# PhiSpel/lettuce

Measured on AMD Instinct MI355X. Metric: MLUPS (million lattice updates/s) D3Q19 256³ TGV; achieved HBM GB/s vs peak, higher is better.
Workload: dtype f32; 1 GPU; TaylorGreenVortex3D D3Q19 BGK fp32 256x256x256 (16777216 nodes per GPU), Re=1600 Ma=0.1; parallelism=single GPU

## Files before the change

### lettuce_amd/csrc/api.hip

```cpp
#include <hip/hip_runtime.h>
#include <stdarg.h>
#include <stdio.h>
#include <string.h>

#include <algorithm>
#include <cmath>
#include <new>
#include <type_traits>

#include "dispatch.hpp"
#include "kernels.hpp"
#include "lettuce_hip.h"

namespace {

thread_local char g_error[512] = "";

int fail(int code, const char *fmt, ...) {
  va_list ap;
  va_start(ap, fmt);
  vsnprintf(g_error, sizeof g_error, fmt, ap);
  va_end(ap);
  return code;
}
// ... 1250 lines not shown
  return aux(p, 0, f, nullptr, u0, nullptr, s, 1.0, 1.0, nullptr, (owned + 6) * plane);
}
int lt_slab_enstrophy(lt_plan *p, const void *u_ext, double u_scale, double inv_dx, double *out, void *s) {
  if (const int rc = slab_plan_ok(p, "lt_slab_enstrophy")) return rc;
  if (!out || !u_ext) return fail(LT_ERR_INVALID, "null output / velocity field");
  return aux(p, 8, nullptr, nullptr, const_cast<void *>(u_ext), out, s, u_scale, inv_dx);
}
int lt_slab_mass_interior(lt_plan *p, const void *f, const uint8_t *mask, int32_t z_begin, int32_t nz_global,
                          double *out, void *s) {
  if (const int rc = slab_plan_ok(p, "lt_slab_mass_interior")) return rc;
  if (!out) return fail(LT_ERR_INVALID, "null output");
  const int owned = p->interior_end - p->interior_begin;
  if (z_begin < 0 || nz_global < 1 || z_begin + owned > nz_global)
    return fail(LT_ERR_INVALID, "planes [%d, %d) of %d", z_begin, z_begin + owned, nz_global);
  return aux(p, 9, f, nullptr, nullptr, out, s, 1.0, 1.0, mask, 0, z_begin, nz_global);
}

int lt_plan_kernel_info(lt_plan *p, int32_t *vec, int32_t *tpb, int64_t *blocks) {
  if (!p) return fail(LT_ERR_INVALID, "null plan");
  if (vec) *vec = 1;
  if (tpb) *tpb = lt::kThreads;
  if (blocks) {
    const long long nodes = (long long)p->n0 * p->n1 * (p->interior_end - p->interior_begin);
    *blocks = (nodes + lt::kThreads - 1) / lt::kThreads;
  }
  return LT_OK;
}

const char *lt_plan_kernel_name(lt_plan *p) {
  if (!p) return "";
  int mode = (two_step_wanted(p) || p->desc.ghost_planes == 2) ? lt::kFusedTwice : lt::kFused;
  if (many_step_wanted(p)) mode = lt::kFusedMany;
  if (mode == lt::kFusedTwice && !has_kernel(p->unit, kernel_selector(p, mode))) mode = lt::kFused;
  const lt::StepArgs a = kernel_selector(p, mode);
  if (!p->unit.name(a, lt::NameBuf{p->kernel_name, sizeof p->kernel_name})) p->kernel_name[0] = 0;
  return p->kernel_name;
}

int lt_slab_crossing(lt_plan *p, int32_t direction, int32_t *q_out, int32_t *n_out) {
  if (!p || !n_out) return fail(LT_ERR_INVALID, "null argument");
  const lt::QList ql = crossing(p, direction);
  *n_out = ql.n;
  if (q_out) for (int k = 0; k < ql.n; ++k) q_out[k] = ql.q[k];
  return LT_OK;
}
int lt_slab_pack(lt_plan *p, const void *f, int64_t plane, int32_t direction, void *buf, void *s) {
  return pack(p, true, const_cast<void *>(f), plane, direction, buf, s);
}
int lt_slab_unpack(lt_plan *p, void *f, int64_t plane, int32_t direction, const void *buf, void *s) {
  return pack(p, false, f, plane, direction, const_cast<void *>(buf), s);
}

int lt_probe_copy(void *dst, const void *src, int64_t n_bytes, int32_t cache_policy,
                  int32_t max_blocks, void *stream) {
  if (!dst || !src || n_bytes < 16 || n_bytes % 16 != 0 || (uintptr_t)dst % 16 || (uintptr_t)src % 16)
    return fail(LT_ERR_INVALID, "probe copy needs 16-byte aligned buffers and size");
  const size_t n = (size_t)n_bytes / 16;
  size_t grid = (n + 255) / 256;
  if (max_blocks > 0 && grid > (size_t)max_blocks) grid = (size_t)max_blocks;
  hipStream_t s = static_cast<hipStream_t>(stream);
  const probe_f4 *sp = static_cast<const probe_f4 *>(src);
  probe_f4 *dp = static_cast<probe_f4 *>(dst);
  switch (cache_policy) {
    case 0: hipLaunchKernelGGL(probe_copy_kernel<0>, dim3((unsigned)grid), dim3(256), 0, s, sp, dp, n); break;
    case 1: hipLaunchKernelGGL(probe_copy_kernel<1>, dim3((unsigned)grid), dim3(256), 0, s, sp, dp, n); break;
    case 2: hipLaunchKernelGGL(probe_copy_kernel<2>, dim3((unsigned)grid), dim3(256), 0, s, sp, dp, n); break;
    case 3: hipLaunchKernelGGL(probe_copy_kernel<3>, dim3((unsigned)grid), dim3(256), 0, s, sp, dp, n); break;
// ... 494 lines not shown
```

### lettuce_amd/csrc/dispatch.hpp

```cpp
#pragma once
#include <hip/hip_runtime.h>
#include <stddef.h>
#include <stdint.h>

namespace lt {

enum StepMode { kFused = 0, kCollideOnly = 1, kStreamOnly = 2, kFusedTwice = 3, kFusedMany = 4 };

constexpr int kCollNone = 0, kCollBgk = 1, kCollKbc = 2, kCollSmagorinsky = 3, kCollForce = 4, kCollTrt = 8,
              kCollRegularized = 9, kCollMrt = 10, kCollMrtLallemand = 11;
constexpr int kCollIncompressible = 16;
constexpr bool coll_incompressible(int coll) { return (coll & kCollIncompressible) != 0; }
constexpr bool coll_mrt(int coll) { return coll == kCollMrt || coll == kCollMrtLallemand; }
constexpr bool coll_forced(int coll) {
  return (coll & ~kCollIncompressible) == (kCollBgk | kCollForce) || coll == (kCollSmagorinsky | kCollForce);
}
constexpr int coll_base(int coll) { return coll_forced(coll) ? coll & ~kCollForce : coll; }

struct StepArgs {
  const void *in;
  void *out;
  int n0, n1, n2;
  long long stride_in, stride_out;
  int p_begin, planes;
// ... 65 lines not shown
#define LT_UNIT_d3q19_f32 D3Q19, float,  19, 3, 0, 1
#define LT_UNIT_d3q19_f64 D3Q19, double, 19, 3, 0, 0
#define LT_UNIT_d3q27_f32 D3Q27, float,  27, 3, 1, 0
#define LT_UNIT_d3q27_f64 D3Q27, double, 27, 3, 1, 0
#define LT_UNIT_d1q3_f32  D1Q3,  float,   3, 1, 0, 0
#define LT_UNIT_d1q3_f64  D1Q3,  double,  3, 1, 0, 0
#define LT_UNIT_d3q15_f32 D3Q15, float,  15, 3, 0, 0
#define LT_UNIT_d3q15_f64 D3Q15, double, 15, 3, 0, 0
#define LT_UNITS(X)                                                                                  \
  X(d2q9_f32) X(d2q9_f64) X(d3q19_f32) X(d3q19_f64) X(d3q27_f32) X(d3q27_f64) X(d1q3_f32) X(d1q3_f64) \
  X(d3q15_f32) X(d3q15_f64)
#define LT_FIELD(name, tag) LT_FIELD_A(name, tag)
#define LT_FIELD_A(name, tag) LT_FIELD_B(name, LT_UNIT_##tag)
#define LT_FIELD_B(name, ...) LT_FIELD_##name(__VA_ARGS__)
#define LT_FIELD_lattice(s, t, q, d, kbc, roles) s
#define LT_FIELD_scalar(s, t, q, d, kbc, roles) t
#define LT_FIELD_q(s, t, q, d, kbc, roles) q
#define LT_FIELD_d(s, t, q, d, kbc, roles) d
#define LT_FIELD_kbc(s, t, q, d, kbc, roles) kbc
#define LT_FIELD_roles(s, t, q, d, kbc, roles) roles

#define LT_DECLARE_UNIT(tag)                                   \
  int step_##tag(const StepArgs &);                            \
  int aux_##tag(const AuxArgs &);                              \
  const char *name_##tag(const StepArgs &, const NameBuf &);   \
  int forced_##tag(const StepArgs &, const NameBuf *);         \
  int relax_##tag(const StepArgs &, const NameBuf *);          \
  int outlets_##tag(const StepArgs &, const NameBuf *);        \
  int outlets2_##tag(const StepArgs &, const NameBuf *);       \
  int outlets3_##tag(const StepArgs &, const NameBuf *);       \
  int twice_##tag(const StepArgs &, const NameBuf *);          \
  int smag_##tag(const StepArgs &, const NameBuf *);           \
  int roles_##tag(const StepArgs &, const NameBuf *);          \
  int mrt_##tag(const StepArgs &, const NameBuf *);            \
  int mrt_outlets_##tag(const StepArgs &, const NameBuf *);    \
  int incompressible_##tag(const StepArgs &, const NameBuf *); \
  int incompressible_aux_##tag(const AuxArgs &);               \
  int spectrum_##tag(const AuxArgs &);
LT_UNITS(LT_DECLARE_UNIT)

constexpr int kNoKernel = -1;

}
```

### lettuce_amd/csrc/kernels.hpp

```cpp
#pragma once
#include <hip/hip_runtime.h>
#include <stdint.h>

#include "dispatch.hpp"
#include "lattice.hpp"
#include "mrt.hpp"
#include "twostep_roles.hpp"

namespace lt {

constexpr int kThreads = 256;
constexpr int kMaxB = 127;

constexpr int kBounceBack = 1, kEquilibrium = 2, kAbbOutlet = 3;
constexpr int kPressureOutlet = 4;
constexpr int kOutletsP = 4;

template <typename T>
struct BoundaryTable {
  int kind[kMaxB + 1];
  int mem_axis[kMaxB + 1];
  int side[kMaxB + 1];
  int plane[kMaxB + 1];
  int nbr[kMaxB + 1];
// ... 959 lines not shown
  static_assert(VEC == 1 && SHIFT == 0, "one node per thread");
  static_assert(coll_incompressible(COLL) && !coll_forced(COLL), "the incompressible equilibrium is COLL & 16");
  lbm_body<T, S, LAYOUT, COLL, STREAM, COLLIDE, MASKED, TUNE, PACK, ABBD>(p);
}
template <typename T, class S, int LAYOUT, int COLL, bool STREAM, bool COLLIDE, bool MASKED,
          int VEC, int SHIFT, int TUNE = 0, bool PACK = false, int ABBD = 0>
__global__ void __launch_bounds__(kThreads) lbm_kernel(const KParamsFI<T> p) {
  static_assert(VEC == 1 && SHIFT == 0, "one node per thread");
  static_assert(coll_incompressible(COLL) && coll_forced(COLL), "BGK with a body force and the incompressible equilibrium is COLL 21");
  lbm_body<T, S, LAYOUT, COLL, STREAM, COLLIDE, MASKED, TUNE, PACK, ABBD>(p);
}

template <typename T, class S, int LAYOUT, int COLL, bool STREAM, bool COLLIDE, bool MASKED,
          int VEC, int SHIFT, int TUNE = 0, bool PACK = false>
__global__ void __launch_bounds__(kThreads, 4) lbm_kernel_occ4(const KParams<T> p) {
  static_assert(VEC == 1 && SHIFT == 0, "one node per thread");
  lbm_body<T, S, LAYOUT, COLL, STREAM, COLLIDE, MASKED, TUNE, PACK>(p);
}

template <typename T, class S, int T0_, int T1>
struct TwoStep {
  static constexpr int T0 = T0_, H0 = T0 + 2, H1 = T1 + 2;
  static constexpr int NI = H0 * H1;
  static constexpr int NO = T0 * T1;
  static constexpr int THREADS = (NI + 63) / 64 * 64;
  template <int LAYOUT, int E2>
  static constexpr int count() {
    int n = 0;
    for (int q = 0; q < S::Q; ++q) n += MemMap<S, LAYOUT>::e(q, 2) == E2 ? 1 : 0;
    return n;
  }
};

__device__ __forceinline__ void lds_barrier() {
  asm volatile("s_waitcnt lgkmcnt(0)\n\ts_barrier" ::: "memory");
}

template <typename T, class S, int LAYOUT, int COLL, int T0_, int T1, int NPT = 1, int MODE = 0,
          int NPB = NPT, int SCHED = 0>
__global__ void __launch_bounds__((SCHED == 0 ? (TwoStep<T, S, T0_, T1>::NI / NPT + 63) / 64 * 64
                                              : RoleWaves<TwoStep<T, S, T0_, T1>::NI, TwoStep<T, S, T0_, T1>::NO>::THREADS))
lbm2_kernel(const KParams<T> p, const int seg_len) {
  static_assert(!coll_forced(COLL), "kernels with a body force take KParamsF");
#include "twostep_sweep.inc"
}

template <typename T, class S, int LAYOUT, int COLL, int T0_, int T1, int NPT = 1, int MODE = 0,
          int NPB = NPT, int SCHED = 0>
__global__ void __launch_bounds__((TwoStep<T, S, T0_, T1>::NI / NPT + 63) / 64 * 64)
lbm2_kernel(const KParamsF<T> p, const int seg_len) {
  static_assert(coll_forced(COLL), "a body force exists for BGK (5) and Smagorinsky (7)");
#include "twostep_sweep.inc"
}

static __global__ void wait_counter_kernel(const unsigned long long *counter, unsigned long long target,
                                           unsigned *timed_out) {
  const long long t0 = wall_clock64();
  while (__hip_atomic_load(counter, __ATOMIC_RELAXED, __HIP_MEMORY_SCOPE_AGENT) < target) {
    __builtin_amdgcn_s_sleep(127);
    if (wall_clock64() - t0 > 100000000ll) {
      *timed_out = 1u;
      break;
    }
  }
  __atomic_thread_fence(__ATOMIC_ACQUIRE);
}
// ... 447 lines not shown
```

### lettuce_amd/csrc/twostep_masked.hpp

```cpp
#pragma once
#include "kernels.hpp"

namespace lt {

typedef unsigned bufu2 __attribute__((ext_vector_type(2)));

template <typename T> struct BufIO;
template <> struct BufIO<float> {
  static __device__ __forceinline__ float load(__amdgpu_buffer_rsrc_t r, unsigned voff, unsigned soff) {
    return __builtin_bit_cast(float, __builtin_amdgcn_raw_buffer_load_b32(r, (int)voff, (int)soff, 0));
  }
  static __device__ __forceinline__ void store_nt(float v, __amdgpu_buffer_rsrc_t r, unsigned voff, unsigned soff) {
    __builtin_amdgcn_raw_buffer_store_b32(__builtin_bit_cast(unsigned, v), r, (int)voff, (int)soff, 2);
  }
};
template <> struct BufIO<double> {
  static __device__ __forceinline__ double load(__amdgpu_buffer_rsrc_t r, unsigned voff, unsigned soff) {
    return __builtin_bit_cast(double, __builtin_amdgcn_raw_buffer_load_b64(r, (int)voff, (int)soff, 0));
  }
  static __device__ __forceinline__ void store_nt(double v, __amdgpu_buffer_rsrc_t r, unsigned voff, unsigned soff) {
    __builtin_amdgcn_raw_buffer_store_b64(__builtin_bit_cast(bufu2, v), r, (int)voff, (int)soff, 2);
  }
};

template <typename T>
__device__ __forceinline__ __amdgpu_buffer_rsrc_t field_rsrc(const T *field, unsigned bytes) {
  return __builtin_amdgcn_make_buffer_rsrc(const_cast<T *>(field), 0, (int)bytes, 0x00020000);
}

constexpr int kEqCached = 2;
template <typename T, class S, int LAYOUT, int T0, int T1>
constexpr size_t two_step_masked_lds() {
  using B = TwoStep<T, S, T0, T1>;
  return sizeof(T) * ((size_t)B::NI * (4 * B::template count<LAYOUT, 1>() + 3 * B::template count<LAYOUT, 0>() +
                                       3 * B::template count<LAYOUT, -1>()) + (size_t)kEqCached * S::Q);
}

struct MaskedPlanInfo {
  unsigned kinds;
  unsigned fields;
  int eq0, eq1;
  int abb_slot, abb_side, abb_plane, abb_axis;
};
template <typename T>
__device__ __forceinline__ MaskedPlanInfo masked_plan_info(const KParams<T> &p) {
  MaskedPlanInfo m = {0u, 0u, 0, 0, 0, 1, -1, 2};
  int cached = 0;
  for (int slot = 1; slot <= p.nb; ++slot) {
    const int kind = p.bt->kind[slot];
    m.kinds |= (unsigned)kind << (2 * slot);
    if (kind == kEquilibrium) {
      if (p.bt->field[slot]) m.fields |= 1u << slot;
      else if (cached == 0) { m.eq0 = slot; cached = 1; }
      else if (cached == 1) { m.eq1 = slot; cached = 2; }
    }
    if (kind == kAbbOutlet) {
      m.abb_slot = slot; m.abb_side = p.bt->side[slot]; m.abb_plane = p.bt->plane[slot];
      m.abb_axis = p.bt->mem_axis[slot];
    }
  }
  return m;
// ... 302 lines not shown
```

### lettuce_amd/csrc/twostep_roles.hpp

```cpp
#pragma once
#include <type_traits>

#if defined(__HIPCC__)
#define LT_ROLE_FN __host__ __device__ __forceinline__
#else
#define LT_ROLE_FN inline
#endif

namespace lt {

template <int SET>
using RegSet = std::integral_constant<int, SET>;

template <class Load, class Fill, class Sync, class Drain, class Emit>
LT_ROLE_FN void role_sweep(const int s, const int last, Load &&load, Fill &&fill, Sync &&sync, Drain &&drain,
                           Emit &&emit) {
  load(s - 1, RegSet<0>{});
  load(s, RegSet<1>{});
  fill(0, 0, RegSet<0>{});
  load(s + 1, RegSet<0>{});
  fill(1, 1, RegSet<1>{});
  int k = s, r = 1, r3 = 1;
  auto interval = [&](auto cur, auto with_load, auto with_fill) {
    constexpr int CUR = decltype(cur)::value;
// ... 4 lines not shown
    emit(k);
    ++k;
    ++r;
    r3 = r3 == 2 ? 0 : r3 + 1;
  };
  using Yes = std::true_type;
  using No = std::false_type;
  if (s + 2 > last) {
    fill(2, 2, RegSet<0>{});
    interval(RegSet<1>{}, No{}, No{});
    return;
  }
  load(s + 2, RegSet<1>{});
  fill(2, 2, RegSet<0>{});
  for (;;) {
    if (k + 3 > last) { interval(RegSet<1>{}, No{}, Yes{}); break; }
    interval(RegSet<1>{}, Yes{}, Yes{});
    if (k + 3 > last) { interval(RegSet<0>{}, No{}, Yes{}); break; }
    interval(RegSet<0>{}, Yes{}, Yes{});
  }
  while (k < last) interval(RegSet<0>{}, No{}, No{});
}

template <int NI, int NO>
struct RoleWaves {
  static constexpr int PW = (NI + 63) / 64;
  static constexpr int CPB = PW + NO / 64 > 16 ? 2 : 1;
  static constexpr int CW = NO / CPB / 64;
  static constexpr int THREADS = (PW + CW) * 64;
  static_assert(NO % (CPB * 64) == 0, "whole consumer waves");
  static_assert(PW + CW <= 16, "a workgroup has at most 1024 threads");
};

}
```

### lettuce_amd/csrc/twostep_sweep.inc

```
  constexpr bool PACK = MODE == 1;
  static_assert(MODE == 0 || LAYOUT == 1, "edge / signalling launches exist in the slab layout");
  static_assert(NPT == 1 && NPB == 1, "one intermediate and one output node per thread");
  static_assert(SCHED == 0 || (SCHED == 1 && MODE == 0), "separate producer and consumer waves: the plain sweep");
  using B = TwoStep<T, S, T0_, T1>;
  using M = MemMap<S, LAYOUT>;
  constexpr int T0 = B::T0, H0 = B::H0, NI = B::NI, NO = B::NO;
  constexpr int NU = B::template count<LAYOUT, 1>(), NC = B::template count<LAYOUT, 0>(),
                ND = B::template count<LAYOUT, -1>();
  static_assert(COLL == kCollNone || COLL == kCollBgk || COLL == kCollSmagorinsky || coll_forced(COLL) || COLL == kCollTrt ||
                    COLL == kCollRegularized,
                "two-step kernel: streaming only, BGK or Smagorinsky, the latter two also with a body force, TRT, regularised");
  static_assert(COLL == kCollNone || COLL == kCollBgk || (SCHED == 0 && MODE == 0),
                "Smagorinsky, body force, TRT, regularised: the plain one-role sweep only");
  __shared__ T lds_u[4][NU][NI];
  __shared__ T lds_c[3][NC][NI];
  __shared__ T lds_d[2][ND][NI];

  const int tid = threadIdx.x;
  const int tiles0 = p.n0 / T0, tiles1 = p.n1 / T1;
  int b = blockIdx.x;
  const int segs_a = (p.p_end - p.p_begin + seg_len - 1) / seg_len;
  if (MODE == 2) {
    const int tiles = tiles0 * tiles1;
    const int layer = b / tiles, t = b - layer * tiles;
    const int tile = tiles % 8 == 0 ? (t % 8) * (tiles / 8) + t / 8 : t;
    b = (layer == 0 ? segs_a : layer - 1) * tiles + tile;
  } else if (p.nb == 0 && (tiles0 * tiles1) % 8 == 0) {
    const int tiles = tiles0 * tiles1;
    const int layer = b / tiles, t = b - layer * tiles;
    b = layer * tiles + (t % 8) * (tiles / 8) + t / 8;
  } else if (p.nb != 1 && gridDim.x % 8 == 0) {
    b = (b % 8) * (gridDim.x / 8) + b / 8;
  }
  const int t0 = (b % tiles0) * T0; b /= tiles0;
  const int t1 = (b % tiles1) * T1; b /= tiles1;
  const bool second = b >= segs_a;
// ... 4 lines not shown
  unsigned voff[NPT][3][3];
  unsigned out_off[NPB];
  int a_at[NPT];
  int b_at[NPB];
  static_for<NPT>([&](auto kc) {
    constexpr int k = decltype(kc)::value;
    const int ia = tid + k * NI;
    constexpr int inner = T0 * B::H1;
    const int i1 = ia < inner ? ia / T0 : (ia - inner) >> 1;
    const int i0 = ia < inner ? 1 + (ia - i1 * T0) : (((ia - inner) & 1) ? H0 - 1 : 0);
    a_at[k] = i1 * H0 + i0;
    int g0 = t0 + i0 - 1; g0 = g0 < 0 ? g0 + p.n0 : (g0 >= p.n0 ? g0 - p.n0 : g0);
    int g1 = t1 + i1 - 1; g1 = g1 < 0 ? g1 + p.n1 : (g1 >= p.n1 ? g1 - p.n1 : g1);
    const int g0m = g0 == 0 ? p.n0 - 1 : g0 - 1, g0p = g0 == p.n0 - 1 ? 0 : g0 + 1;
    const int g1m = g1 == 0 ? p.n1 - 1 : g1 - 1, g1p = g1 == p.n1 - 1 ? 0 : g1 + 1;
#pragma unroll
    for (int a = 0; a < 3; ++a)
#pragma unroll
      for (int c = 0; c < 3; ++c) {
        const int y = a == 0 ? g1p : (a == 1 ? g1 : g1m);
        const int x = c == 0 ? g0p : (c == 1 ? g0 : g0m);
        voff[k][a][c] = ((unsigned)y * (unsigned)p.n0 + (unsigned)x) * (unsigned)sizeof(T);
      }
  });
  static_for<NPB>([&](auto kc) {
    constexpr int k = decltype(kc)::value;
    const int ib = tid + k * NO;
    const int j1 = ib / T0, j0 = ib - j1 * T0;
    out_off[k] = ((unsigned)(t1 + j1) * (unsigned)p.n0 + (unsigned)(t0 + j0)) * (unsigned)sizeof(T);
    b_at[k] = (j1 + 1) * H0 + (j0 + 1);
  });
  const unsigned plane_nodes = (unsigned)p.n1 * (unsigned)p.n0;

  if constexpr (SCHED == 1) {
    using R = RoleWaves<NI, NO>;
    constexpr int CPB = R::CPB, CT = NO / CPB;
    const int last = s + seg_len < range_end ? s + seg_len : range_end;
    auto sync = [&]() { lds_barrier(); };
    if (__builtin_amdgcn_readfirstlane(tid >> 6) < R::PW) {
      if (!in_a) {
#pragma unroll
        for (int a = 0; a < 3; ++a)
#pragma unroll
          for (int c = 0; c < 3; ++c) voff[0][a][c] = 0u;
      }
      T set0[S::Q][1], set1[S::Q][1];
      auto load = [&](int plane, auto set) {
        T (&dst)[S::Q][1] = decltype(set)::value == 0 ? set0 : set1;
        int g2 = plane, g2m = plane - 1, g2p = plane + 1;
        if (p.wrap2) {
          g2 = plane < 0 ? plane + p.n2 : (plane >= p.n2 ? plane - p.n2 : plane);
          g2m = g2 == 0 ? p.n2 - 1 : g2 - 1;
          g2p = g2 == p.n2 - 1 ? 0 : g2 + 1;
        }
        static_for<S::Q>([&](auto qc) {
          constexpr int q = decltype(qc)::value;
          constexpr int e0 = M::e(q, 0), e1 = M::e(q, 1), e2 = M::e(q, 2);
          const int z = e2 == 0 ? g2 : (e2 > 0 ? g2m : g2p);
          const T *base = p.in + ((long long)q * p.Ni + (long long)((unsigned)z * plane_nodes));
          dst[q][0] = *reinterpret_cast<const T *>(reinterpret_cast<const char *>(base) + voff[0][e1 + 1][e0 + 1]);
        });
        __builtin_amdgcn_sched_barrier(0);
      };
      auto fill = [&](int r, int r3, auto set) {
        T (&src)[S::Q][1] = decltype(set)::value == 0 ? set0 : set1;
        collide_node<T, S, LAYOUT, 1, 0, COLL>(src, p);
        if (in_a) {
          static_for<S::Q>([&](auto qc) {
            constexpr int q = decltype(qc)::value;
            constexpr int e2 = M::e(q, 2), rank = crossing_rank<S, LAYOUT, q>();
            if constexpr (e2 > 0) lds_u[r & 3][rank][a_at[0]] = src[q][0];
            else if constexpr (e2 == 0) lds_c[r3][rank][a_at[0]] = src[q][0];
            else lds_d[r & 1][rank][a_at[0]] = src[q][0];
          });
        }
        __builtin_amdgcn_sched_barrier(0);
      };
      role_sweep(s, last, load, fill, sync, [](int, int) {}, [](int) {});
    } else {
      const int c = tid - R::PW * 64;
      unsigned c_off[CPB];
      int c_at[CPB];
      static_for<CPB>([&](auto kc) {
        constexpr int k = decltype(kc)::value;
        const int ib = c + k * CT;
        const int j1 = ib / T0, j0 = ib - j1 * T0;
        c_off[k] = ((unsigned)(t1 + j1) * (unsigned)p.n0 + (unsigned)(t0 + j0)) * (unsigned)sizeof(T);
        c_at[k] = (j1 + 1) * H0 + (j0 + 1);
      });
      T f[S::Q][CPB];
      auto drain = [&](int r, int r3) {
        static_for<S::Q>([&](auto qc) {
          constexpr int q = decltype(qc)::value;
          constexpr int e0 = M::e(q, 0), e1 = M::e(q, 1), e2 = M::e(q, 2), rank = crossing_rank<S, LAYOUT, q>();
          static_for<CPB>([&](auto kc) {
            constexpr int k = decltype(kc)::value;
            const int at = c_at[k] - e1 * H0 - e0;
            if constexpr (e2 > 0) f[q][k] = lds_u[(r - 1) & 3][rank][at];
            else if constexpr (e2 == 0) f[q][k] = lds_c[r3][rank][at];
            else f[q][k] = lds_d[(r + 1) & 1][rank][at];
          });
        });
      };
      auto emit = [&](int k2) {
        static_for<CPB>([&](auto kc) { collide_node<T, S, LAYOUT, CPB, decltype(kc)::value, COLL>(f, p); });
        static_for<S::Q>([&](auto qc) {
          constexpr int q = decltype(qc)::value;
          T *base = p.out + ((long long)q * p.No + (long long)((unsigned)k2 * plane_nodes));
          static_for<CPB>([&](auto kc) {
            constexpr int k = decltype(kc)::value;
            __builtin_nontemporal_store(f[q][k], reinterpret_cast<T *>(reinterpret_cast<char *>(base) + c_off[k]));
          });
        });
      };
      role_sweep(s, last, [](int, auto) {}, [](int, int, auto) {}, sync, drain, emit);
    }
    return;
  }
  T pre[S::Q][NPT];
  auto load_a = [&](int plane) {
    int g2 = plane, g2m = plane - 1, g2p = plane + 1;
    if (p.wrap2) {
      g2 = plane < 0 ? plane + p.n2 : (plane >= p.n2 ? plane - p.n2 : plane);
      g2m = g2 == 0 ? p.n2 - 1 : g2 - 1;
      g2p = g2 == p.n2 - 1 ? 0 : g2 + 1;
    }
    if (in_a) {
      static_for<S::Q>([&](auto qc) {
        constexpr int q = decltype(qc)::value;
        constexpr int e0 = M::e(q, 0), e1 = M::e(q, 1), e2 = M::e(q, 2);
        const int z = e2 == 0 ? g2 : (e2 > 0 ? g2m : g2p);
        const T *base = p.in + ((long long)q * p.Ni + (long long)((unsigned)z * plane_nodes));
        if constexpr (MODE == 1) {
          constexpr int rank = crossing_rank<S, LAYOUT, q>();
          if constexpr (e2 >= 0) {
            if (p.ghost_lo != nullptr && z < p.lo)
              base = p.ghost_lo + (size_t)(e2 == 0 ? rank : (z == p.lo - 1 ? NC + rank : NC + NU + rank)) * plane_nodes;
          }
          if constexpr (e2 <= 0) {
            if (p.ghost_hi != nullptr && z >= p.hi)
              base = p.ghost_hi + (size_t)(e2 == 0 ? rank : (z == p.hi ? NC + rank : NC + ND + rank)) * plane_nodes;
          }
        }
        static_for<NPT>([&](auto kc) {
          constexpr int k = decltype(kc)::value;
// ... 189 lines not shown
```

### lettuce_amd/csrc/unit.inc

```
#include <cstdio>
#include <algorithm>
#include <type_traits>

#include "dispatch.hpp"
#include "kernels.hpp"
#include "twostep_masked.hpp"
#include "twostep2d.hpp"
#include "spectrum.hpp"

#define LT_CAT_(a, b) a##b
#define LT_CAT(a, b) LT_CAT_(a, b)
#define LT_TAG LT_UNIT
#define LT_S lt::LT_FIELD(lattice, LT_UNIT)
#define LT_T LT_FIELD(scalar, LT_UNIT)
#define LT_IS_3D (LT_FIELD(d, LT_UNIT) == 3)
#define LT_HAS_KBC LT_FIELD(kbc, LT_UNIT)
#define LT_HAS_ROLES LT_FIELD(roles, LT_UNIT)
#define LT_HAS_MRT (LT_FIELD(q, LT_UNIT) == 9 || LT_FIELD(q, LT_UNIT) == 27)

#define LT_PART_main 1
#define LT_PART_sweeps 2
#define LT_PART_roles 3
#define LT_PART_smagorinsky 4
#define LT_PART_forced 5
#define LT_PART_relaxations 6
#define LT_PART_outlets 7
#define LT_PART_outlets2 8
#define LT_PART_outlets3 9
#define LT_PART_mrt 10
#define LT_PART_mrt_outlets 11
#define LT_PART_incompressible 12
#define LT_PART_spectrum 13
#define LT_PART_IS_OUTLETS (LT_PART_IS(outlets) || LT_PART_IS(outlets2) || LT_PART_IS(outlets3) || LT_PART_IS(mrt_outlets))
#define LT_PART_IS(name) (LT_CAT(LT_PART_, LT_PART) == LT_PART_##name)
#if LT_PART_IS(main)
#define LT_ONE_STEP 1
#define LT_SWEEP 0
#elif LT_PART_IS(sweeps)
#define LT_ONE_STEP 0
#define LT_SWEEP 1
#elif LT_PART_IS(roles)
#define LT_ONE_STEP 0
#define LT_SWEEP 1
#elif LT_PART_IS(smagorinsky)
#define LT_ONE_STEP 1
#define LT_SWEEP 0
#elif LT_PART_IS(forced)
#define LT_ONE_STEP 1
#define LT_SWEEP 1
#elif LT_PART_IS(relaxations)
#define LT_ONE_STEP 1
#define LT_SWEEP 1
#elif LT_PART_IS_OUTLETS || LT_PART_IS(mrt) || LT_PART_IS(incompressible)
#define LT_ONE_STEP 1
#define LT_SWEEP 0
#elif LT_PART_IS(spectrum)
#define LT_ONE_STEP 0
#define LT_SWEEP 0
#else
#error "LT_PART: main, sweeps, roles, smagorinsky, forced, relaxations, outlets, outlets2, outlets3, mrt, mrt_outlets, incompressible or spectrum"
#endif
#if (LT_PART_IS(mrt) || LT_PART_IS(mrt_outlets)) && !LT_HAS_MRT
#error "the MRT collision exists on D2Q9 and D3Q27"
#endif
#if LT_PART_IS(spectrum) && LT_FIELD(d, LT_UNIT) < 2
#error "the energy spectrum exists in 2-D and 3-D"
#endif

namespace lt {
namespace {

using S = LT_S;
using T = LT_T;
constexpr size_t kTwicePerNode = sizeof(T) * 3 * S::Q;
constexpr int kTwiceW = 256 / (int)sizeof(T);
constexpr int kTwiceR = kTwicePerNode * (kTwiceW + 2) * 10 <= 160 * 1024 ? 8
                        : (sizeof(T) == 4 && kTwicePerNode * (kTwiceW + 2) * 6 <= 160 * 1024 ? 4 : 0);

template <int COLL>
using ParamsOfQuadratic = std::conditional_t<coll_mrt(COLL), KParamsM<T>, std::conditional_t<coll_forced(COLL), KParamsF<T>, KParams<T>>>;
template <int COLL>
using ParamsOf = std::conditional_t<coll_incompressible(COLL), std::conditional_t<coll_forced(COLL), KParamsFI<T>, KParamsI<T>>,
                                    ParamsOfQuadratic<COLL>>;
template <class P>
P params_of(const StepArgs &a, int n2) {
  P p{};
  p.in = static_cast<const T *>(a.in);
  p.out = static_cast<T *>(a.out);
  p.n0 = a.n0; p.n1 = a.n1; p.n2 = n2;
  p.nv0 = a.n0;
  p.p_begin = a.p_begin;
  p.p_stride = a.p_stride;
  p.wrap2 = a.wrap2;
// ... 168 lines not shown
  return kNoKernel;
}
#endif

#endif

#if LT_SWEEP
template <int LAYOUT, int COLL, int T0, int T1, int MODE = 0, int SCHED = 0>
int launch_twice(const StepArgs &a, const NameBuf *name) {
  if constexpr (S::D == 3 && T0 > 0 &&
                (COLL == kCollNone || COLL == kCollBgk ||
                 ((COLL == kCollSmagorinsky || COLL == (kCollBgk | kCollForce) || COLL == kCollTrt || COLL == kCollRegularized) &&
                  S::Q == 19 && sizeof(T) == 4 && MODE == 0 && SCHED == 0))) {
    using B = TwoStep<T, S, T0, T1>;
    if (name) return kernel_name(*name, "lbm2_kernel", LAYOUT, COLL, T0, T1, 1, MODE, 1, elided(SCHED));
    if (a.n0 % T0 != 0 || a.n1 % T1 != 0 || a.seg_len < 1 || a.masked || a.planes < 1 || a.p_stride != 1 ||
        (long long)a.n0 * a.n1 * (long long)sizeof(T) >= (1ll << 32))
      return kNoKernel;
    if (MODE == 2 && (!a.signal || a.planes2 < 2 || a.planes2 > a.seg_len || a.seg_len < 2)) return kNoKernel;
    using P = ParamsOf<COLL>;
    P p = params_of<P>(a, a.n2);
    p.p_end = a.p_begin + a.planes;
    p.p_begin2 = a.p_begin2;
    p.p_end2 = a.p_begin2 + a.planes2;
    if constexpr (coll_forced(COLL)) set_force<LAYOUT>(p, a);
    p.nb = a.shift == 3 ? 1 : (a.shift == 4 ? 2 : 0);
    p.signal = MODE == 2 ? a.signal : nullptr;
    p.edge_first = MODE == 2 ? 1 : 0;
    p.ghost_lo = static_cast<const T *>(a.ghost_lo);
    p.ghost_hi = static_cast<const T *>(a.ghost_hi);
    p.lo = a.interior_begin; p.hi = a.interior_end;
    const unsigned grid = (unsigned)((a.n0 / T0) * (a.n1 / T1) * ((a.planes + a.seg_len - 1) / a.seg_len +
                                                                   (a.planes2 + a.seg_len - 1) / a.seg_len));
    constexpr int threads = SCHED ? RoleWaves<B::NI, B::NO>::THREADS : (B::NI + 63) / 64 * 64;
    void (*kern)(const P, const int) = lbm2_kernel<T, S, LAYOUT, COLL, T0, T1, 1, MODE, 1, SCHED>;
    hipLaunchKernelGGL(kern, dim3(grid), dim3(threads), 0, a.stream, p, a.seg_len);
    return (int)hipGetLastError();
  } else {
    return kNoKernel;
  }
}

int sweep(const StepArgs &a, const NameBuf *name) {
  constexpr int W = kTwiceW, R = kTwiceR;
  if constexpr (R > 0) {
#if LT_PART_IS(roles)
    if (a.layout == 0) return launch_twice<0, kCollBgk, W, R, 0, 1>(a, name);
    return launch_twice<1, kCollBgk, W, R, 0, 1>(a, name);
#elif LT_PART_IS(forced)
    if (a.masked || a.pack_lo || a.pack_hi || a.signal) return kNoKernel;
    if (a.layout == 0 && a.coll == (kCollBgk | kCollForce)) return launch_twice<0, kCollBgk | kCollForce, W, R>(a, name);
    if (a.layout == 1 && a.coll == (kCollBgk | kCollForce)) return launch_twice<1, kCollBgk | kCollForce, W, R>(a, name);
#elif LT_PART_IS(relaxations)
    if (a.masked || a.pack_lo || a.pack_hi || a.signal) return kNoKernel;
    if (a.layout == 0 && a.coll == kCollTrt) return launch_twice<0, kCollTrt, W, R>(a, name);
    if (a.layout == 1 && a.coll == kCollTrt) return launch_twice<1, kCollTrt, W, R>(a, name);
    if (a.layout == 0 && a.coll == kCollRegularized) return launch_twice<0, kCollRegularized, W, R>(a, name);
    if (a.layout == 1 && a.coll == kCollRegularized) return launch_twice<1, kCollRegularized, W, R>(a, name);
#else
    const int coll = a.coll;
#if LT_HAS_ROLES
    if (coll == kCollBgk && a.shift != 6 && (a.layout == 0 || !(a.pack_lo || a.pack_hi || a.signal)))
      return LT_CAT(roles_, LT_TAG)(a, name);
#endif
    if (a.layout == 0 && coll == kCollNone) return launch_twice<0, kCollNone, W, R>(a, name);
    if (a.layout == 0 && coll == kCollBgk) return launch_twice<0, kCollBgk, W, R>(a, name);
    if (a.layout == 0 && coll == kCollSmagorinsky) return launch_twice<0, kCollSmagorinsky, W, R>(a, name);
    if (coll == kCollSmagorinsky && (a.pack_lo || a.pack_hi || a.signal)) return kNoKernel;
    if (a.layout == 1 && (a.pack_lo || a.pack_hi)) {
      if (coll == kCollNone) return launch_twice<1, kCollNone, W, R, 1>(a, name);
      if (coll == kCollBgk) return launch_twice<1, kCollBgk, W, R, 1>(a, name);
    }
    if (a.layout == 1 && a.signal) {
      if (coll == kCollNone) return launch_twice<1, kCollNone, W, R, 2>(a, name);
      if (coll == kCollBgk) return launch_twice<1, kCollBgk, W, R, 2>(a, name);
    }
    if (a.layout == 1 && coll == kCollNone) return launch_twice<1, kCollNone, W, R>(a, name);
    if (a.layout == 1 && coll == kCollBgk) return launch_twice<1, kCollBgk, W, R>(a, name);
    if (a.layout == 1 && coll == kCollSmagorinsky) return launch_twice<1, kCollSmagorinsky, W, R>(a, name);
#endif
  }
// ... 242 lines not shown
        hipLaunchKernelGGL(finish_sum_kernel<false>, dim3(1), dim3(kThreads), 0, a.stream, a.partial,
                           a.reduce_blocks, a.out);
        break;
      } else {
        return kNoKernel;
      }
    default:
      return kNoKernel;
  }
  return (int)hipGetLastError();
}

#endif

}

#if LT_PART_IS(main)
int LT_CAT(step_, LT_TAG)(const StepArgs &a) { return dispatch(a, nullptr); }

const char *LT_CAT(name_, LT_TAG)(const StepArgs &a, const NameBuf &name) {
  return dispatch(a, &name) == 0 ? name.s : nullptr;
}

int LT_CAT(aux_, LT_TAG)(const AuxArgs &a) {
#if LT_IS_3D
  if (a.layout == 1) return aux_impl<1>(a);
#endif
  return aux_impl<0>(a);
}
#elif LT_PART_IS(sweeps)
int LT_CAT(twice_, LT_TAG)(const StepArgs &a, const NameBuf *name) { return sweep(a, name); }
#elif LT_PART_IS(roles)
int LT_CAT(roles_, LT_TAG)(const StepArgs &a, const NameBuf *name) { return sweep(a, name); }
#elif LT_PART_IS(smagorinsky)
int LT_CAT(smag_, LT_TAG)(const StepArgs &a, const NameBuf *name) { return one_step_of<kCollSmagorinsky>(a, name); }
#elif LT_PART_IS(forced)
int LT_CAT(forced_, LT_TAG)(const StepArgs &a, const NameBuf *name) {
  if (a.mode == kFusedTwice) return S::D == 3 ? sweep(a, name) : kNoKernel;
  if (a.coll == (kCollBgk | kCollForce)) return one_step_of<kCollBgk | kCollForce>(a, name);
  if (a.coll == (kCollSmagorinsky | kCollForce)) return one_step_of<kCollSmagorinsky | kCollForce>(a, name);
  return kNoKernel;
}
#elif LT_PART_IS(relaxations)
int LT_CAT(relax_, LT_TAG)(const StepArgs &a, const NameBuf *name) {
  if (a.mode == kFusedTwice) return S::D == 3 ? sweep(a, name) : kNoKernel;
  if (a.mode != kFused && a.mode != kCollideOnly) return kNoKernel;
  if (a.coll == kCollTrt) return one_step_of<kCollTrt>(a, name);
  if (a.coll == kCollRegularized) return one_step_of<kCollRegularized>(a, name);
  return kNoKernel;
}
#elif LT_PART_IS(outlets)
int LT_CAT(outlets_, LT_TAG)(const StepArgs &a, const NameBuf *name) {
  if (a.mode != kFused && a.mode != kCollideOnly) return kNoKernel;
  switch (a.coll) {
    case kCollNone: return pressure_outlets_of<kCollNone>(a, name);
    case kCollBgk: return pressure_outlets_of<kCollBgk>(a, name);
#if LT_HAS_KBC
    case kCollKbc: return pressure_outlets_of<kCollKbc>(a, name);
#endif
    case kCollSmagorinsky: case kCollTrt: case kCollRegularized: return LT_CAT(outlets2_, LT_TAG)(a, name);
    case kCollBgk | kCollForce: case kCollSmagorinsky | kCollForce: return LT_CAT(outlets3_, LT_TAG)(a, name);
#if LT_HAS_MRT
    case kCollMrt: case kCollMrtLallemand: return LT_CAT(mrt_outlets_, LT_TAG)(a, name);
#endif
    default: return kNoKernel;
  }
// ... 76 lines not shown
```

Baseline: 68680 MLUPS.

## Use buffer loads/stores and trimmed LDS writes in role-split two-step BGK sweep

For the producer/consumer role-split two-step kernel in the SoA layout, global loads and non-temporal stores now go through AMD buffer resources with scalar (uniform) offsets instead of 64-bit flat addressing. This is meant to cut per-lane address arithmetic and VGPR pressure. Edge producer waves also skip LDS writes for populations that their consumers never read. A new compilation part carries the buffer variant, guarded by a check that the field fits in 32-bit offsets, with a fallback (SCHED=2) that keeps flat addressing. The kernel-name query now fills in grid dims and strides so the addressability guard can be evaluated.

```diff
diff --git a/lettuce_amd/csrc/api.hip b/lettuce_amd/csrc/api.hip
--- a/lettuce_amd/csrc/api.hip
+++ b/lettuce_amd/csrc/api.hip
@@ -1306,7 +1306,9 @@
   int mode = (two_step_wanted(p) || p->desc.ghost_planes == 2) ? lt::kFusedTwice : lt::kFused;
   if (many_step_wanted(p)) mode = lt::kFusedMany;
   if (mode == lt::kFusedTwice && !has_kernel(p->unit, kernel_selector(p, mode))) mode = lt::kFused;
-  const lt::StepArgs a = kernel_selector(p, mode);
+  lt::StepArgs a = kernel_selector(p, mode);
+  a.n0 = p->n0; a.n1 = p->n1; a.n2 = p->n2;
+  a.stride_in = a.stride_out = p->res[0] ? p->res_stride : p->pop_stride;
   if (!p->unit.name(a, lt::NameBuf{p->kernel_name, sizeof p->kernel_name})) p->kernel_name[0] = 0;
   return p->kernel_name;
 }
diff --git a/lettuce_amd/csrc/dispatch.hpp b/lettuce_amd/csrc/dispatch.hpp
--- a/lettuce_amd/csrc/dispatch.hpp
+++ b/lettuce_amd/csrc/dispatch.hpp
@@ -121,6 +121,7 @@
   int twice_##tag(const StepArgs &, const NameBuf *);          \
   int smag_##tag(const StepArgs &, const NameBuf *);           \
   int roles_##tag(const StepArgs &, const NameBuf *);          \
+  int roles_trim_##tag(const StepArgs &, const NameBuf *);     \
   int mrt_##tag(const StepArgs &, const NameBuf *);            \
   int mrt_outlets_##tag(const StepArgs &, const NameBuf *);    \
   int incompressible_##tag(const StepArgs &, const NameBuf *); \
diff --git a/lettuce_amd/csrc/kernels.hpp b/lettuce_amd/csrc/kernels.hpp
--- a/lettuce_amd/csrc/kernels.hpp
+++ b/lettuce_amd/csrc/kernels.hpp
@@ -1015,6 +1015,31 @@
   }
 };
 
+typedef unsigned bufu2 __attribute__((ext_vector_type(2)));
+
+template <typename T> struct BufIO;
+template <> struct BufIO<float> {
+  static __device__ __forceinline__ float load(__amdgpu_buffer_rsrc_t r, unsigned voff, unsigned soff) {
+    return __builtin_bit_cast(float, __builtin_amdgcn_raw_buffer_load_b32(r, (int)voff, (int)soff, 0));
+  }
+  static __device__ __forceinline__ void store_nt(float v, __amdgpu_buffer_rsrc_t r, unsigned voff, unsigned soff) {
+    __builtin_amdgcn_raw_buffer_store_b32(__builtin_bit_cast(unsigned, v), r, (int)voff, (int)soff, 2);
+  }
+};
+template <> struct BufIO<double> {
+  static __device__ __forceinline__ double load(__amdgpu_buffer_rsrc_t r, unsigned voff, unsigned soff) {
+    return __builtin_bit_cast(double, __builtin_amdgcn_raw_buffer_load_b64(r, (int)voff, (int)soff, 0));
+  }
+  static __device__ __forceinline__ void store_nt(double v, __amdgpu_buffer_rsrc_t r, unsigned voff, unsigned soff) {
+    __builtin_amdgcn_raw_buffer_store_b64(__builtin_bit_cast(bufu2, v), r, (int)voff, (int)soff, 2);
+  }
+};
+
+template <typename T>
+__device__ __forceinline__ __amdgpu_buffer_rsrc_t field_rsrc(const T *field, unsigned bytes) {
+  return __builtin_amdgcn_make_buffer_rsrc(const_cast<T *>(field), 0, (int)bytes, 0x00020000);
+}
+
 __device__ __forceinline__ void lds_barrier() {
   asm volatile("s_waitcnt lgkmcnt(0)\n\ts_barrier" ::: "memory");
 }
diff --git a/lettuce_amd/csrc/twostep_masked.hpp b/lettuce_amd/csrc/twostep_masked.hpp
--- a/lettuce_amd/csrc/twostep_masked.hpp
+++ b/lettuce_amd/csrc/twostep_masked.hpp
@@ -2,31 +2,6 @@
 #include "kernels.hpp"
 
 namespace lt {
-
-typedef unsigned bufu2 __attribute__((ext_vector_type(2)));
-
-template <typename T> struct BufIO;
-template <> struct BufIO<float> {
-  static __device__ __forceinline__ float load(__amdgpu_buffer_rsrc_t r, unsigned voff, unsigned soff) {
-    return __builtin_bit_cast(float, __builtin_amdgcn_raw_buffer_load_b32(r, (int)voff, (int)soff, 0));
-  }
-  static __device__ __forceinline__ void store_nt(float v, __amdgpu_buffer_rsrc_t r, unsigned voff, unsigned soff) {
-    __builtin_amdgcn_raw_buffer_store_b32(__builtin_bit_cast(unsigned, v), r, (int)voff, (int)soff, 2);
-  }
-};
-template <> struct BufIO<double> {
-  static __device__ __forceinline__ double load(__amdgpu_buffer_rsrc_t r, unsigned voff, unsigned soff) {
-    return __builtin_bit_cast(double, __builtin_amdgcn_raw_buffer_load_b64(r, (int)voff, (int)soff, 0));
-  }
-  static __device__ __forceinline__ void store_nt(double v, __amdgpu_buffer_rsrc_t r, unsigned voff, unsigned soff) {
-    __builtin_amdgcn_raw_buffer_store_b64(__builtin_bit_cast(bufu2, v), r, (int)voff, (int)soff, 2);
-  }
-};
-
-template <typename T>
-__device__ __forceinline__ __amdgpu_buffer_rsrc_t field_rsrc(const T *field, unsigned bytes) {
-  return __builtin_amdgcn_make_buffer_rsrc(const_cast<T *>(field), 0, (int)bytes, 0x00020000);
-}
 
 constexpr int kEqCached = 2;
 template <typename T, class S, int LAYOUT, int T0, int T1>
diff --git a/lettuce_amd/csrc/twostep_roles.hpp b/lettuce_amd/csrc/twostep_roles.hpp
--- a/lettuce_amd/csrc/twostep_roles.hpp
+++ b/lettuce_amd/csrc/twostep_roles.hpp
@@ -60,4 +60,17 @@
   static_assert(PW + CW <= 16, "a workgroup has at most 1024 threads");
 };
 
+inline bool role_field_within_32_bits(int q, int esize, long long nodes, long long stride) {
+  const long long widest = stride > nodes ? stride : nodes;
+  if (q <= 0 || esize <= 0 || nodes < 0) return false;
+  return widest <= ((1ll << 32) - 1) / ((long long)q * esize);
 }
+inline bool role_buffer_addressable(int q, int esize, long long n0, long long n1, long long n2, long long stride_in,
+                                    long long stride_out) {
+  if (n0 < 0 || n1 < 0 || n2 < 0) return false;
+  if (n0 > 0 && n1 > 0 && n2 > (1ll << 40) / n0 / n1) return false;
+  const long long nodes = n0 * n1 * n2;
+  return role_field_within_32_bits(q, esize, nodes, stride_in) && role_field_within_32_bits(q, esize, nodes, stride_out);
+}
+
+}
diff --git a/lettuce_amd/csrc/twostep_sweep.inc b/lettuce_amd/csrc/twostep_sweep.inc
--- a/lettuce_amd/csrc/twostep_sweep.inc
+++ b/lettuce_amd/csrc/twostep_sweep.inc
@@ -1,7 +1,7 @@
   constexpr bool PACK = MODE == 1;
   static_assert(MODE == 0 || LAYOUT == 1, "edge / signalling launches exist in the slab layout");
   static_assert(NPT == 1 && NPB == 1, "one intermediate and one output node per thread");
-  static_assert(SCHED == 0 || (SCHED == 1 && MODE == 0), "separate producer and consumer waves: the plain sweep");
+  static_assert(SCHED == 0 || ((SCHED == 1 || SCHED == 2) && MODE == 0), "separate producer and consumer waves: the plain sweep");
   using B = TwoStep<T, S, T0_, T1>;
   using M = MemMap<S, LAYOUT>;
   constexpr int T0 = B::T0, H0 = B::H0, NI = B::NI, NO = B::NO;
@@ -72,18 +72,24 @@
   });
   const unsigned plane_nodes = (unsigned)p.n1 * (unsigned)p.n0;
 
-  if constexpr (SCHED == 1) {
+  if constexpr (SCHED != 0) {
+    constexpr bool BUF = SCHED == 1 && LAYOUT == 0;
     using R = RoleWaves<NI, NO>;
     constexpr int CPB = R::CPB, CT = NO / CPB;
     const int last = s + seg_len < range_end ? s + seg_len : range_end;
     auto sync = [&]() { lds_barrier(); };
-    if (__builtin_amdgcn_readfirstlane(tid >> 6) < R::PW) {
+    auto uniform = [](unsigned v) { return (unsigned)__builtin_amdgcn_readfirstlane((int)v); };
+    const unsigned plane_bytes = plane_nodes * (unsigned)sizeof(T);
+    const int wave = __builtin_amdgcn_readfirstlane(tid >> 6);
+    if (wave < R::PW) {
       if (!in_a) {
 #pragma unroll
         for (int a = 0; a < 3; ++a)
 #pragma unroll
           for (int c = 0; c < 3; ++c) voff[0][a][c] = 0u;
       }
+      const unsigned pop_in = BUF ? uniform((unsigned)(p.Ni * (long long)sizeof(T))) : 0u;
+      const __amdgpu_buffer_rsrc_t in_r = field_rsrc(p.in, (unsigned)S::Q * pop_in);
       T set0[S::Q][1], set1[S::Q][1];
       auto load = [&](int plane, auto set) {
         T (&dst)[S::Q][1] = decltype(set)::value == 0 ? set0 : set1;
@@ -97,26 +103,44 @@
           constexpr int q = decltype(qc)::value;
           constexpr int e0 = M::e(q, 0), e1 = M::e(q, 1), e2 = M::e(q, 2);
           const int z = e2 == 0 ? g2 : (e2 > 0 ? g2m : g2p);
-          const T *base = p.in + ((long long)q * p.Ni + (long long)((unsigned)z * plane_nodes));
-          dst[q][0] = *reinterpret_cast<const T *>(reinterpret_cast<const char *>(base) + voff[0][e1 + 1][e0 + 1]);
+          if constexpr (BUF) {
+            dst[q][0] = BufIO<T>::load(in_r, voff[0][e1 + 1][e0 + 1], uniform((unsigned)q * pop_in + (unsigned)z * plane_bytes));
+          } else {
+            const T *base = p.in + ((long long)q * p.Ni + (long long)((unsigned)z * plane_nodes));
+            dst[q][0] = *reinterpret_cast<const T *>(reinterpret_cast<const char *>(base) + voff[0][e1 + 1][e0 + 1]);
+          }
         });
         __builtin_amdgcn_sched_barrier(0);
       };
-      auto fill = [&](int r, int r3, auto set) {
-        T (&src)[S::Q][1] = decltype(set)::value == 0 ? set0 : set1;
-        collide_node<T, S, LAYOUT, 1, 0, COLL>(src, p);
-        if (in_a) {
-          static_for<S::Q>([&](auto qc) {
-            constexpr int q = decltype(qc)::value;
-            constexpr int e2 = M::e(q, 2), rank = crossing_rank<S, LAYOUT, q>();
-            if constexpr (e2 > 0) lds_u[r & 3][rank][a_at[0]] = src[q][0];
-            else if constexpr (e2 == 0) lds_c[r3][rank][a_at[0]] = src[q][0];
-            else lds_d[r & 1][rank][a_at[0]] = src[q][0];
-          });
-        }
-        __builtin_amdgcn_sched_barrier(0);
-      };
-      role_sweep(s, last, load, fill, sync, [](int, int) {}, [](int) {});
+      auto produce = [&](auto trim) {
+        constexpr int TRIM = decltype(trim)::value;
+        auto fill = [&](int r, int r3, auto set) {
+          T (&src)[S::Q][1] = decltype(set)::value == 0 ? set0 : set1;
+          collide_node<T, S, LAYOUT, 1, 0, COLL>(src, p);
+          if (in_a) {
+            static_for<S::Q>([&](auto qc) {
+              constexpr int q = decltype(qc)::value;
+              constexpr int e0 = M::e(q, 0), e1 = M::e(q, 1), e2 = M::e(q, 2), rank = crossing_rank<S, LAYOUT, q>();
+              constexpr bool READ = TRIM == 0 || (TRIM == 1 && e1 == 1) || (TRIM == 2 && e1 == -1) || (TRIM == 3 && e0 != 0);
+              if constexpr (READ) {
+                if constexpr (e2 > 0) lds_u[r & 3][rank][a_at[0]] = src[q][0];
+                else if constexpr (e2 == 0) lds_c[r3][rank][a_at[0]] = src[q][0];
+                else lds_d[r & 1][rank][a_at[0]] = src[q][0];
+              }
+            });
+          }
+          __builtin_amdgcn_sched_barrier(0);
+        };
+        role_sweep(s, last, load, fill, sync, [](int, int) {}, [](int) {});
+      };
+      if constexpr (BUF && T0 == 64 && R::PW == B::H1 + 1) {
+        if (wave == 0) produce(std::integral_constant<int, 1>{});
+        else if (wave == B::H1 - 1) produce(std::integral_constant<int, 2>{});
+        else if (wave == B::H1) produce(std::integral_constant<int, 3>{});
+        else produce(std::integral_constant<int, 0>{});
+      } else {
+        produce(std::integral_constant<int, 0>{});
+      }
     } else {
       const int c = tid - R::PW * 64;
       unsigned c_off[CPB];
@@ -128,6 +152,8 @@
         c_off[k] = ((unsigned)(t1 + j1) * (unsigned)p.n0 + (unsigned)(t0 + j0)) * (unsigned)sizeof(T);
         c_at[k] = (j1 + 1) * H0 + (j0 + 1);
       });
+      const unsigned pop_out = BUF ? uniform((unsigned)(p.No * (long long)sizeof(T))) : 0u;
+      const __amdgpu_buffer_rsrc_t out_r = field_rsrc(p.out, (unsigned)S::Q * pop_out);
       T f[S::Q][CPB];
       auto drain = [&](int r, int r3) {
         static_for<S::Q>([&](auto qc) {
@@ -146,11 +172,19 @@
         static_for<CPB>([&](auto kc) { collide_node<T, S, LAYOUT, CPB, decltype(kc)::value, COLL>(f, p); });
         static_for<S::Q>([&](auto qc) {
           constexpr int q = decltype(qc)::value;
-          T *base = p.out + ((long long)q * p.No + (long long)((unsigned)k2 * plane_nodes));
-          static_for<CPB>([&](auto kc) {
-            constexpr int k = decltype(kc)::value;
-            __builtin_nontemporal_store(f[q][k], reinterpret_cast<T *>(reinterpret_cast<char *>(base) + c_off[k]));
-          });
+          if constexpr (BUF) {
+            const unsigned soff = uniform((unsigned)q * pop_out + (unsigned)k2 * plane_bytes);
+            static_for<CPB>([&](auto kc) {
+              constexpr int k = decltype(kc)::value;
+              BufIO<T>::store_nt(f[q][k], out_r, c_off[k], soff);
+            });
+          } else {
+            T *base = p.out + ((long long)q * p.No + (long long)((unsigned)k2 * plane_nodes));
+            static_for<CPB>([&](auto kc) {
+              constexpr int k = decltype(kc)::value;
+              __builtin_nontemporal_store(f[q][k], reinterpret_cast<T *>(reinterpret_cast<char *>(base) + c_off[k]));
+            });
+          }
         });
       };
       role_sweep(s, last, [](int, auto) {}, [](int, int, auto) {}, sync, drain, emit);
diff --git a/lettuce_amd/csrc/unit.inc b/lettuce_amd/csrc/unit.inc
--- a/lettuce_amd/csrc/unit.inc
+++ b/lettuce_amd/csrc/unit.inc
@@ -31,6 +31,7 @@
 #define LT_PART_mrt_outlets 11
 #define LT_PART_incompressible 12
 #define LT_PART_spectrum 13
+#define LT_PART_roles_trim 14
 #define LT_PART_IS_OUTLETS (LT_PART_IS(outlets) || LT_PART_IS(outlets2) || LT_PART_IS(outlets3) || LT_PART_IS(mrt_outlets))
 #define LT_PART_IS(name) (LT_CAT(LT_PART_, LT_PART) == LT_PART_##name)
 #if LT_PART_IS(main)
@@ -39,7 +40,7 @@
 #elif LT_PART_IS(sweeps)
 #define LT_ONE_STEP 0
 #define LT_SWEEP 1
-#elif LT_PART_IS(roles)
+#elif LT_PART_IS(roles) || LT_PART_IS(roles_trim)
 #define LT_ONE_STEP 0
 #define LT_SWEEP 1
 #elif LT_PART_IS(smagorinsky)
@@ -58,7 +59,7 @@
 #define LT_ONE_STEP 0
 #define LT_SWEEP 0
 #else
-#error "LT_PART: main, sweeps, roles, smagorinsky, forced, relaxations, outlets, outlets2, outlets3, mrt, mrt_outlets, incompressible or spectrum"
+#error "LT_PART: main, sweeps, roles, roles_trim, smagorinsky, forced, relaxations, outlets, outlets2, outlets3, mrt, mrt_outlets, incompressible or spectrum"
 #endif
 #if (LT_PART_IS(mrt) || LT_PART_IS(mrt_outlets)) && !LT_HAS_MRT
 #error "the MRT collision exists on D2Q9 and D3Q27"
@@ -293,6 +294,9 @@
     p.lo = a.interior_begin; p.hi = a.interior_end;
     const unsigned grid = (unsigned)((a.n0 / T0) * (a.n1 / T1) * ((a.planes + a.seg_len - 1) / a.seg_len +
                                                                    (a.planes2 + a.seg_len - 1) / a.seg_len));
+    if constexpr (SCHED == 1 && LAYOUT == 0) {
+      if (!role_buffer_addressable(S::Q, (int)sizeof(T), a.n0, a.n1, a.n2, a.stride_in, a.stride_out)) return kNoKernel;
+    }
     constexpr int threads = SCHED ? RoleWaves<B::NI, B::NO>::THREADS : (B::NI + 63) / 64 * 64;
     void (*kern)(const P, const int) = lbm2_kernel<T, S, LAYOUT, COLL, T0, T1, 1, MODE, 1, SCHED>;
     hipLaunchKernelGGL(kern, dim3(grid), dim3(threads), 0, a.stream, p, a.seg_len);
@@ -306,8 +310,14 @@
   constexpr int W = kTwiceW, R = kTwiceR;
   if constexpr (R > 0) {
 #if LT_PART_IS(roles)
+    if (a.layout == 0) {
+      if (role_buffer_addressable(S::Q, (int)sizeof(T), a.n0, a.n1, a.n2, a.stride_in, a.stride_out))
+        return LT_CAT(roles_trim_, LT_TAG)(a, name);
+      return launch_twice<0, kCollBgk, W, R, 0, 2>(a, name);
+    }
+    return launch_twice<1, kCollBgk, W, R, 0, 1>(a, name);
+#elif LT_PART_IS(roles_trim)
     if (a.layout == 0) return launch_twice<0, kCollBgk, W, R, 0, 1>(a, name);
-    return launch_twice<1, kCollBgk, W, R, 0, 1>(a, name);
 #elif LT_PART_IS(forced)
     if (a.masked || a.pack_lo || a.pack_hi || a.signal) return kNoKernel;
     if (a.layout == 0 && a.coll == (kCollBgk | kCollForce)) return launch_twice<0, kCollBgk | kCollForce, W, R>(a, name);
@@ -616,6 +626,8 @@
 int LT_CAT(twice_, LT_TAG)(const StepArgs &a, const NameBuf *name) { return sweep(a, name); }
 #elif LT_PART_IS(roles)
 int LT_CAT(roles_, LT_TAG)(const StepArgs &a, const NameBuf *name) { return sweep(a, name); }
+#elif LT_PART_IS(roles_trim)
+int LT_CAT(roles_trim_, LT_TAG)(const StepArgs &a, const NameBuf *name) { return sweep(a, name); }
 #elif LT_PART_IS(smagorinsky)
 int LT_CAT(smag_, LT_TAG)(const StepArgs &a, const NameBuf *name) { return one_step_of<kCollSmagorinsky>(a, name); }
 #elif LT_PART_IS(forced)
```

Measured after the change: 69180 MLUPS, median of 3. Within noise of the previous version (+0.7%).
